# hellosunking/Microcket

Measured on AMD Instinct MI355X. Metric: read-pairs/sec through sam2pairs+dedup (150 bp PE, hg38 names, SAM text resident in HBM), higher is better.
Workload: dtype u8; 1 GPU; C2: 100 M 150 bp PE Micro-C read pairs, hg38, one MI355X -- 100000000 synthetic 150 bp PE read pairs per GPU, hg38 chromosome names, 1 lane(s), unc mode, sam=no, seed 20260105, one step = one pass over the whole resident data set + duplicate marking of the reported pairs on (chr1,pos1,chr2,pos2,strands) + per-chromosome-pair counts; preset=C2, pairs_per_gpu=100000001, sam_bytes_per_gpu=94584442002, block_groups=2097152, blocks=48, parallelism=shard1: independent read-group shards, no data-path collective

## Files before the change

### microcket_amd/csrc/mkt_capi.cpp

```cpp
#include <hip/hip_runtime.h>
#include <stdarg.h>
#include <stdio.h>
#include <stdlib.h>
#include <string.h>
#include <algorithm>
#include <string>
#include <utility>
#include <chrono>
#include <condition_variable>
#include <deque>
#include <mutex>
#include <thread>
#include <vector>

#include "../../include/mkt.h"
#include "mkt_launch.h"

using namespace mkt;

static const size_t kMaxBlock = ((size_t)1 << 31) - 65536;

static thread_local std::string g_create_error;

struct mkt_ctx {
// ... 236 lines not shown

static int ensure_sc_list(mkt_ctx* c, size_t need);

static void set_dims_from_avg(mkt_ctx* c, double bytes_per_line) {
    c->dims_probed = true;
    c->halo_widened = 0;
    if (c->cfg == CFG_SMALL || c->p.tiles != MKT_TILES_AUTO) return;
    c->dims = lean_dims(bytes_per_line);
    if (getenv("MKT_DEBUG_SYNC")) fprintf(stderr, "tile geometry: %.1f bytes per line -> tile %u, halos %u / %u\n", bytes_per_line, c->dims.tile, c->dims.hb, c->dims.hf);
}
static bool shrink_dims(mkt_ctx* c) {
    if (c->cfg == CFG_SMALL || c->dims.tile <= 2048u) return false;
    auto f = [](uint32_t x, uint32_t lo) { uint32_t y = ((uint32_t)(x * 0.6) + 15u) & ~15u; return y < lo ? lo : y; };
    c->dims.tile = f(c->dims.tile, 2048u); c->dims.hb = f(c->dims.hb, 256u); c->dims.hf = f(c->dims.hf, 512u);
    return true;
}
static bool widen_halos(mkt_ctx* c) {
    if (c->cfg == CFG_SMALL || c->halo_widened >= 2) return false;
    const TileDims mx = max_dims();
    auto f = [](uint32_t x, uint32_t hi) { uint32_t y = ((uint32_t)(x * 1.5) + 15u) & ~15u; return y > hi ? hi : y; };
    const uint32_t hb = f(c->dims.hb, mx.hb), hf = f(c->dims.hf, mx.hf);
    const uint32_t delta = (hb - c->dims.hb) + (hf - c->dims.hf);
    if (delta == 0 || c->dims.tile < delta + 2048u) return false;
    c->dims.tile -= delta; c->dims.hb = hb; c->dims.hf = hf;
    ++c->halo_widened;
    if (getenv("MKT_DEBUG_SYNC")) fprintf(stderr, "tile geometry: halos widened -> tile %u, halos %u / %u\n", c->dims.tile, c->dims.hb, c->dims.hf);
    return true;
}
static bool adapt_geometry(mkt_ctx* c, const BlockResult& r) {
    if (c->p.tiles != MKT_TILES_AUTO || c->p.ordered) return false;
    if (r.tiles >= 1000 && (uint64_t)r.pad2 * 500 > r.tiles && widen_halos(c)) return true;
    if (r.tiles >= 8 && (uint64_t)(r.pad - r.pad2) * 8 > r.tiles) return shrink_dims(c);
    return false;
}
static double probe_device_lines(mkt_ctx* c, const uint8_t* d_text, size_t n) {
    const size_t look = n < ((size_t)1 << 20) ? n : ((size_t)1 << 20);
    if (!look) return 0;
    if (!c->d_probe) {
        if (hipMalloc((void**)&c->d_probe, sizeof(unsigned long long)) != hipSuccess) return 0;
        if (hipHostMalloc((void**)&c->h_probe, sizeof(unsigned long long), hipHostMallocDefault) != hipSuccess) return 0;
    }
    if (hipMemsetAsync(c->d_probe, 0, sizeof(unsigned long long), c->stream) != hipSuccess) return 0;
    if (launch_count_newlines(d_text, look, c->d_probe, c->stream) != hipSuccess) return 0;
    if (hipMemcpyAsync(c->h_probe, c->d_probe, sizeof(unsigned long long), hipMemcpyDeviceToHost, c->stream) != hipSuccess) return 0;
    if (hipStreamSynchronize(c->stream) != hipSuccess) return 0;
    return *c->h_probe ? (double)look / (double)*c->h_probe : (double)look;
}
static void smaller_geometry(mkt_ctx* c, const uint8_t* d_text, size_t n) {
    if (c->cfg != CFG_SMALL && d_text) {
        const double avg = probe_device_lines(c, d_text, n);
        const TileDims d = avg > 0 ? lean_dims(avg) : c->dims;
        if (d.tile < c->dims.tile) { c->dims = d; return; }
    }
    if (!shrink_dims(c)) { c->cfg = CFG_SMALL; c->dims = small_dims(); }
}

struct StreamOut { uint8_t* gp; size_t gp_cap; uint8_t* gs; size_t gs_cap; hipEvent_t k0, k1, done; };
static int enqueue_block(mkt_ctx* c, const uint8_t* d_text, size_t n, int cfg, const TileDims& dims, size_t slot, const StreamOut* so = nullptr) {
    if (((uintptr_t)d_text & 15u) != 0) return fail(c, MKT_E_ARG, "block text must be 16-byte aligned");
    if (n >= kMaxBlock) return fail(c, MKT_E_ARG, "block of %zu bytes: must be < 2 GiB - 64 KiB", n);
    const uint32_t ntiles = num_tiles((uint32_t)n, dims.tile);
    int rc = ensure_ws(c, ntiles);
    if (rc) return rc;
    if ((rc = ensure_dev(c, &c->d_pairs, &c->pairs_cap, n / 3 + 65536))) return rc;
    if (c->P.write_sam && (rc = ensure_dev(c, &c->d_sam, &c->sam_cap, n + n / 4 + 65536))) return rc;
    if (!c->d_sc && (rc = ensure_sc_list(c, 1))) return rc;
    KArgs a;
    memset(&a, 0, sizeof a);
    uint8_t* w = c->d_ws;
    a.text = d_text; a.n = (uint32_t)n; a.ntiles = ntiles; a.dims = dims; a.P = c->P;
    a.descA = (uint64_t*)w; w += (size_t)ntiles * 8;
    a.descB = (uint64_t*)w; w += (size_t)ntiles * 8;
    a.descC = (uint64_t*)w; w += (size_t)ntiles * 8;
    a.tile_last = (TileLast*)w; w += (size_t)ntiles * sizeof(TileLast);
    a.tile_groups = (uint64_t*)w; w += (size_t)ntiles * sizeof(uint64_t);
    a.defer_list = (uint32_t*)w;
    w = c->d_ws + ws_tiles_bytes(ntiles);
    a.cur = (RegionCur*)w; w += kMaxRegions * sizeof(RegionCur);
    a.ticket = (uint32_t*)w;
    a.defer_count = (uint32_t*)(w + 64);
    uint32_t* ticket2 = (uint32_t*)(w + 128);
    a.last_tile = (int*)(w + 192);
    a.scan_ticket = (uint32_t*)(w + 224);
    w += 256;
    a.scan_desc = (uint64_t*)w; w += 1024 * sizeof(uint64_t);
    if ((ntiles + finish_chunk_tiles() - 1) / finish_chunk_tiles() > 1024) return fail(c, MKT_E_ARG, "block has too many tiles for the finish scan");
    a.res = (BlockResult*)w;
    a.ordered = c->p.ordered ? 1 : 0;
    a.run = c->d_run;
    a.nregions = c->p.ordered ? 1 : kMaxRegions;
    {
        const size_t need = (size_t)a.nregions * ((n / 256 / (size_t)a.nregions) * 2 + 1024);
        if (c->sc_tmp_cap < need) {
            if (c->d_sc_tmp) { if ((rc = sync_all(c))) return rc; HIPCHK(c, hipFree(c->d_sc_tmp)); }
            c->d_sc_tmp = nullptr; c->sc_tmp_cap = 0;
            HIPCHK(c, hipMalloc((void**)&c->d_sc_tmp, need * sizeof(uint64_t)));
            c->sc_tmp_cap = need;
        }
    }
    a.pairs_rcap = (c->pairs_cap / a.nregions) & ~(uint64_t)15;
    a.sam_rcap = c->P.write_sam ? ((c->sam_cap / a.nregions) & ~(uint64_t)15) : 0;
    a.sc_rcap = c->sc_tmp_cap / a.nregions;
    a.out.pairs = c->d_pairs; a.out.pairs_cap = c->pairs_cap;
    a.out.sam = c->d_sam; a.out.sam_cap = c->P.write_sam ? c->sam_cap : 0;
    a.out.sc = c->d_sc_tmp; a.out.sc_cap = c->sc_tmp_cap;
    a.sc_list = c->d_sc; a.sc_list_cap = c->sc_cap;
    if (c->p.extensions & MKT_EXT_KEYS) {
        if (!c->d_chr) { HIPCHK(c, hipMalloc((void**)&c->d_chr, sizeof(ChrTab))); HIPCHK(c, hipMemsetAsync(c->d_chr, 0, sizeof(ChrTab), c->stream)); }
        const size_t per = (n / 64 / (size_t)a.nregions) * 2 + 4096, need = per * a.nregions;
        if (c->keys_raw_cap < need) {
            if (c->d_keys_raw) { if ((rc = sync_all(c))) return rc; HIPCHK(c, hipFree(c->d_keys_raw)); }
            c->d_keys_raw = nullptr; c->keys_raw_cap = 0;
            HIPCHK(c, hipMalloc((void**)&c->d_keys_raw, need * sizeof(KeyRec)));
            c->keys_raw_cap = need;
        }
        const double per_byte = c->key_density > 0 ? (c->key_density * 2 < 1.0 / 64 ? c->key_density * 2 : 1.0 / 64) : 1.0 / 64;
        const size_t want = (size_t)c->acc.emitted + (size_t)((double)(c->bytes_unsynced + n) * per_byte) + 65536;
        if (c->key_list_cap < want) {
            size_t ncap = c->key_list_cap ? c->key_list_cap * 2 : ((size_t)1 << 22);
            while (ncap < want) ncap *= 2;
            KeyRec* nl = nullptr;
            HIPCHK(c, hipStreamSynchronize(c->stream));
            HIPCHK(c, hipMalloc((void**)&nl, ncap * sizeof(KeyRec)));
            if (c->d_key_list) { HIPCHK(c, hipMemcpy(nl, c->d_key_list, c->key_list_cap * sizeof(KeyRec), hipMemcpyDeviceToDevice)); HIPCHK(c, hipFree(c->d_key_list)); }
            c->d_key_list = nl; c->key_list_cap = ncap;
        }
        a.keys_rcap = c->keys_raw_cap / a.nregions;
        a.out.keys = c->d_keys_raw; a.out.keys_cap = c->keys_raw_cap; a.out.chr = c->d_chr;
        a.out.key_lanes = (c->p.extensions & MKT_EXT_LANES) ? 1u : 0u;
        a.key_list = c->d_key_list; a.key_list_cap = c->key_list_cap;
    }
#if defined(MKT_STAMPS)
    if (!c->d_stamps) { HIPCHK(c, hipMalloc((void**)&c->d_stamps, 16 * sizeof(unsigned long long))); HIPCHK(c, hipMemset(c->d_stamps, 0, 16 * sizeof(unsigned long long))); }
    a.stamps = getenv("MKT_NO_STAMPS") ? nullptr : c->d_stamps;
    { const char* e = getenv("MKT_DEBUG_STOP"); a.debug_stop = e ? atoi(e) : 0; }
#endif
    HIPCHK(c, hipMemsetAsync(c->d_ws, 0, ws_bytes_for(ntiles), c->stream));
    hipEvent_t e0, e1;
    if (so) { e0 = so->k0; e1 = so->k1; }
    else {
        HIPCHK(c, hipEventCreate(&e0));
        HIPCHK(c, hipEventCreate(&e1));
        c->ev.push_back(e0); c->ev.push_back(e1); c->ev_bytes.push_back(n);
    }
    const uint32_t max_wgs = fast_max_workgroups(cfg);
    int grid = (int)(ntiles < max_wgs ? ntiles : max_wgs);
    const bool lean = !c->p.ordered && cfg != CFG_SMALL && !c->no_lean;
    HIPCHK(c, hipEventRecord(e0, c->stream));
    if (lean) {
        HIPCHK(c, launch_fast(a, cfg, grid, c->stream));
        HIPCHK(c, hipEventRecord(e1, c->stream));
        KArgs b = a;
        b.use_list = 1; b.ticket = ticket2;
        HIPCHK(c, launch_tiles(b, cfg, ntiles < 96u ? (int)ntiles : 96, c->stream));
    } else {
        HIPCHK(c, launch_tiles(a, cfg, grid, c->stream));
        HIPCHK(c, hipEventRecord(e1, c->stream));
    }
    HIPCHK(c, launch_finish(a, c->stream));
    if (so) {
        const uint64_t prc = a.nregions > 1 ? a.pairs_rcap : 0, src_ = a.nregions > 1 ? a.sam_rcap : 0;
        HIPCHK(c, launch_gather(a.res, c->d_pairs, prc, so->gp, so->gp_cap, 0, n / 8, c->stream));
        if (c->P.write_sam) HIPCHK(c, launch_gather(a.res, c->d_sam, src_, so->gs, so->gs_cap, 1, n, c->stream));
    }
    HIPCHK(c, hipMemcpyAsync(&c->h_res[slot], a.res, sizeof(BlockResult), hipMemcpyDeviceToHost, c->stream));
    if (so) HIPCHK(c, hipEventRecord(so->done, c->stream));
// ... 1091 lines not shown
```

### microcket_amd/csrc/mkt_kernels.hip

```cpp
#include <hip/hip_runtime.h>
#include <type_traits>
#include "mkt_launch.h"

namespace mkt {

constexpr int NT = 256;
constexpr uint64_t FLAG_AGG = 1ull << 62, FLAG_PREFIX = 2ull << 62, PAYLOAD = (1ull << 62) - 1;
constexpr uint32_t LOOKBACK_SPIN_LIMIT = 1u << 22;

struct ScanScratch { uint64_t a[NT / 64], b[NT / 64]; };

#if defined(MKT_STAMPS)
#define STAMP_DECL() unsigned long long stamp_prev_ = 0, stamp_acc_[16] = {0, 0, 0, 0, 0, 0, 0, 0, 0, 0, 0, 0, 0, 0, 0, 0}
#define STAMP(k)                                                                        \
    do {                                                                                \
        if (tid == 0 && a.stamps) {                                                     \
            const unsigned long long now_ = __builtin_amdgcn_s_memtime();               \
            if ((k) > 0) stamp_acc_[(k)] += now_ - stamp_prev_;                         \
            stamp_prev_ = now_;                                                         \
        }                                                                               \
    } while (0)
#define STAMP_FLUSH(t0_)                                                                \
    do {                                                                                \
        if ((t0_) == 0 && a.stamps) for (int k_ = 1; k_ < 16; ++k_) if (stamp_acc_[k_]) atomicAdd(&a.stamps[k_], stamp_acc_[k_]); \
// ... 101 lines not shown
    const uint32_t y = x & 0x7F7F7F7Fu;
    return ~((y + 0x5F5F5F5Fu) | x) & 0x80808080u;
}
__device__ inline uint32_t pack16(uint32_t f0, uint32_t f1, uint32_t f2, uint32_t f3) {
    const uint32_t lo = __builtin_amdgcn_udot4(f1, 0x80402010u, __builtin_amdgcn_udot4(f0, 0x08040201u, 0u, false), false);
    const uint32_t hi = __builtin_amdgcn_udot4(f3, 0x80402010u, __builtin_amdgcn_udot4(f2, 0x08040201u, 0u, false), false);
    return (lo >> 7) | ((hi >> 7) << 8);
}

__device__ inline uint64_t lookback(uint64_t* desc, uint32_t t, uint64_t agg, uint32_t* err_word) {
    const int lane = threadIdx.x & 63;
    if (t == 0) {
        if (lane == 0) __hip_atomic_store(&desc[0], FLAG_PREFIX | agg, __ATOMIC_RELAXED, __HIP_MEMORY_SCOPE_AGENT);
        return 0;
    }
    if (lane == 0) __hip_atomic_store(&desc[t], FLAG_AGG | agg, __ATOMIC_RELAXED, __HIP_MEMORY_SCOPE_AGENT);
    uint64_t excl = 0;
    int64_t j = (int64_t)t - 1;
    uint32_t spins = 0;
    for (;;) {
        const int64_t idx = j - lane;
        uint64_t w = FLAG_PREFIX;
        if (idx >= 0) w = __hip_atomic_load(&desc[idx], __ATOMIC_RELAXED, __HIP_MEMORY_SCOPE_AGENT);
        const uint32_t flag = (uint32_t)(w >> 62);
        const uint64_t m_prefix = __ballot(flag == 2);
        const uint64_t m_invalid = __ballot(flag == 0);
        const int first = m_prefix ? __builtin_ctzll(m_prefix) : 64;
        const uint64_t needed = first >= 63 ? ~0ull : ((1ull << (first + 1)) - 1);
        if (m_invalid & needed) {
            if (++spins > LOOKBACK_SPIN_LIMIT) { if (lane == 0) atomicOr(err_word, (uint32_t)E_LOOKBACK); break; }
            __builtin_amdgcn_s_sleep(4);
            continue;
        }
        uint64_t c = lane <= first ? (w & PAYLOAD) : 0;
#pragma unroll
        for (int d = 32; d >= 1; d >>= 1) c += shfl_xor64(c, d);
        excl += c;
        if (first < 64) break;
        j -= 64;
    }
    if (lane == 0) __hip_atomic_store(&desc[t], FLAG_PREFIX | ((excl + agg) & PAYLOAD), __ATOMIC_RELAXED, __HIP_MEMORY_SCOPE_AGENT);
    return excl;
}

__device__ inline uint32_t claim_ranges(const KArgs& a, uint32_t region, const TileSums& sums, TileSums& base,
                                        uint32_t& region_pair0, uint32_t& region_sam0, OutPtrs& lim) {
    RegionCur* cur = a.cur + region;
    uint32_t err = 0;
    const uint64_t p0 = (uint64_t)region * a.pairs_rcap, s0 = (uint64_t)region * a.sam_rcap, c0 = (uint64_t)region * a.sc_rcap;
    unsigned long long oa = 0, ob = 0;
    if (sums.pair_bytes | sums.emitted) oa = atomicAdd(&cur->a, (unsigned long long)sums.pair_bytes | ((unsigned long long)sums.emitted << kCurShift));
    if (sums.sam_bytes | sums.sc) ob = atomicAdd(&cur->b, (unsigned long long)sums.sam_bytes | ((unsigned long long)sums.sc << kCurShift));
    const uint64_t op = oa & kCurLow, os = ob & kCurLow, oc = ob >> kCurShift;
    if (op + sums.pair_bytes > a.pairs_rcap) err |= E_PAIRS_CAP;
    if (os + sums.sam_bytes > a.sam_rcap) err |= E_SAM_CAP;
    if (oc + sums.sc > a.sc_rcap) err |= E_SC_CAP;
    base.pair_bytes = (uint32_t)(p0 + op); base.sam_bytes = s0 + os; base.sc = (uint32_t)(c0 + oc);
    base.emitted = (uint32_t)((uint64_t)region * a.keys_rcap + (oa >> kCurShift));
    lim.keys_cap = a.keys_rcap ? ((uint64_t)region * a.keys_rcap + ((oa >> kCurShift) + sums.emitted <= a.keys_rcap ? a.keys_rcap : 0)) : 0;
    region_pair0 = (uint32_t)p0; region_sam0 = (uint32_t)s0;
    lim.pairs_cap = err & E_PAIRS_CAP ? 0 : p0 + a.pairs_rcap;
    lim.sam_cap = err & E_SAM_CAP ? 0 : s0 + a.sam_rcap;
    lim.sc_cap = err & E_SC_CAP ? 0 : c0 + a.sc_rcap;
    return err;
}

template <class Cfg>
__global__ __launch_bounds__(NT) void k_tiles(KArgs a) {
    __shared__ TileState<Cfg> st;
    __shared__ ScanScratch scan;
    __shared__ uint32_t s_tile;
    constexpr int NVEC = (Cfg::W + 15) / 16;
    constexpr int NM16 = Cfg::MW * 4;
    constexpr int VPT = (NVEC + NT - 1) / NT;
    constexpr int IPT = (Cfg::LCAP + NT - 1) / NT;
    const int tid = threadIdx.x;
    const Params P = a.P;
    const uint32_t n = a.n;
    __shared__ OutPtrs s_out;
    const uint32_t region = a.nregions > 1 ? (blockIdx.x & (uint32_t)(a.nregions - 1)) : 0u;
    uint16_t* nlmask = reinterpret_cast<uint16_t*>(st.u.m.nlm);
    uint16_t* wsmask = reinterpret_cast<uint16_t*>(st.u.m.wsm);
    STAMP_DECL();

    for (;;) {
        if (tid == 0) {
            s_out = a.out;
            uint32_t k = atomicAdd(a.ticket, 1u);
            if (a.use_list) k = k < *a.defer_count ? a.defer_list[k] : 0xFFFFFFFFu;
            s_tile = k;
            tile_reset(st);
        }
        __syncthreads();
        const uint32_t t = s_tile;
        if (t >= a.ntiles) break;
        STAMP(0);
        const TileGeom G = tile_geom(t, n, a.dims);
        const uint32_t wlen = G.w1 - G.w0;
        const uint32_t nvec = (wlen + 15u) >> 4;
        const TextView tv = tile_view(st, a.text, n, G);

        constexpr int SPT = (NM16 + NT - 1) / NT;
        uint4 xs[SPT];
#pragma unroll
        for (int q = 0; q < SPT; ++q) {
            const uint32_t v = (uint32_t)tid + (uint32_t)q * NT;
            const uint32_t go = G.w0 + (v << 4);
            xs[q] = *reinterpret_cast<const uint4*>(a.text + ((v < nvec && go + 16u <= n) ? go : 0u));
        }
#pragma unroll
        for (int q = 0; q < SPT; ++q) {
            const uint32_t v = (uint32_t)tid + (uint32_t)q * NT;
            if (v >= (uint32_t)NM16) continue;
            uint32_t mnl = 0, mws = 0;
            if (v < nvec) {
                const uint32_t go = G.w0 + (v << 4);
                uint4 x;
                if (go + 16u <= n) {
                    x = xs[q];
                } else {
                    uint32_t w[4] = {0, 0, 0, 0};
                    for (uint32_t b = 0; go + b < n; ++b) w[b >> 2] |= (uint32_t)a.text[go + b] << ((b & 3u) * 8u);
                    x = make_uint4(w[0], w[1], w[2], w[3]);
                }
                *reinterpret_cast<uint4*>(&st.win[v << 4]) = x;
                mnl = nl_bits(x.x) | (nl_bits(x.y) << 4) | (nl_bits(x.z) << 8) | (nl_bits(x.w) << 12);
                mws = ws_bits(x.x) | (ws_bits(x.y) << 4) | (ws_bits(x.z) << 8) | (ws_bits(x.w) << 12);
                const uint32_t r0 = v << 4;
                if (r0 + 16u > wlen) {
                    const uint32_t keep = wlen - r0;
                    mnl &= (1u << keep) - 1u; mws &= (1u << keep) - 1u;
                }
            } else if (v == nvec && (v << 4) < (uint32_t)(Cfg::W + 16)) {
                *reinterpret_cast<uint4*>(&st.win[v << 4]) = make_uint4(0, 0, 0, 0);
            }
            nlmask[v] = (uint16_t)mnl;
            wsmask[v] = (uint16_t)mws;
        }
        __syncthreads();
        STAMP(1);

        {
            uint64_t cnt = 0, dummy = 0, total, td;
            const uint32_t v0 = tid * VPT;
            auto line_bits = [&](uint32_t v) -> uint32_t {
                uint32_t m = nlmask[v];
                const uint32_t r0 = v << 4;
                if (r0 + 16u > wlen - 1u) { const uint32_t keep = wlen - 1u > r0 ? wlen - 1u - r0 : 0u; m &= keep >= 16u ? 0xFFFFu : ((1u << keep) - 1u); }
                return m;
            };
            for (uint32_t k = 0; k < (uint32_t)VPT; ++k) if (v0 + k < nvec) cnt += __popc(line_bits(v0 + k));
            uint64_t ex = cnt;
            block_exscan2(ex, dummy, total, td, scan);
            const uint32_t lead = G.w0 == 0 ? 1u : 0u;
            const uint32_t NL = (uint32_t)total + lead;
            if (NL > (uint32_t)Cfg::LCAP) {
                if (tid == 0) { lds_or(&st.err, E_LINE_TABLE); st.NL = 0; st.first_idx = 0; st.end_idx = 0; }
            } else {
                uint32_t idx = (uint32_t)ex + lead;
                for (uint32_t k = 0; k < (uint32_t)VPT; ++k) {
                    if (v0 + k >= nvec) break;
                    uint32_t m = line_bits(v0 + k);
                    while (m) {
                        const uint32_t b = __builtin_ctz(m);
                        st.off[idx++] = G.w0 + ((v0 + k) << 4) + b + 1u;
                        m &= m - 1u;
// ... 423 lines not shown
        }
        if (total && st.base.pair_bytes + total <= s_out.pairs_cap) {
            const auto& g = st.u.g;
            for (uint32_t e = (ltid + (uint32_t)(NTW / 2)) & (uint32_t)(NTW - 1); e < st.sums.emitted; e += NTW) {
                const uint32_t i = g.em_idx[e];
                fast_emit_line(st, g.g_slot[i], g.g_plen[i], dst + g.x_pair[i]);
            }
        }
        __syncthreads();
        STAMP(11);
        if (tid < (int)C_COUNT) wg_cnt[tid] += st.cnt[tid];
        if (tid == 0 && (st.abn >> 8)) atomicOr(&a.res->err, st.abn >> 8);
        const bool sam_copy = P.write_sam && st.sums.sam_bytes && st.base.sam_bytes + st.sums.sam_bytes <= s_out.sam_cap;
        uint32_t* eo = st.rc.f.pos;
        uint32_t* es = st.rc.f.rclip;
        uint32_t E = 0;
        if (sam_copy) {
            E = (uint32_t)(__popcll(st.m_emit[0]) + __popcll(st.m_emit[1]) + __popcll(st.m_emit[2]) + __popcll(st.m_emit[3]));
            for (uint32_t i = first_idx + (uint32_t)tid; i < NLe; i += NTW) {
                if (!mask_bit(st.m_emit, i)) continue;
                uint32_t k = (uint32_t)__popcll(st.m_emit[i >> 6] & ((1ull << (i & 63u)) - 1ull));
                for (uint32_t w = 0; w < (i >> 6); ++w) k += (uint32_t)__popcll(st.m_emit[w]);
                eo[k] = st.u.g.x_sam[i];
                es[k] = st.goff[i];
            }
            if (tid == 0) eo[E] = (uint32_t)st.sums.sam_bytes;
        }
        if (P.write_sam) __syncthreads();
        if (sam_copy && E) {
            const uint32_t total = (uint32_t)st.sums.sam_bytes;
            uint8_t* dbase = s_out.sam + st.base.sam_bytes;
            const uint8_t* tbase = a.text + G.w0;
            auto line_of = [&](uint32_t d) {
                uint32_t lo = 0, hi = E - 1u;
                while (lo < hi) { const uint32_t mid = (lo + hi + 1u) >> 1; if (eo[mid] <= d) lo = mid; else hi = mid - 1u; }
                return lo;
            };
            const uint32_t head0 = (uint32_t)((16u - ((uintptr_t)dbase & 15u)) & 15u);
            const uint32_t head = head0 < total ? head0 : total;
            const uint32_t nv = (total - head) >> 4, tail0 = head + (nv << 4);
            if ((uint32_t)tid < head) { const uint32_t k = line_of((uint32_t)tid); *MKT_GLOBAL(uint8_t, dbase + tid) = tbase[es[k] + (uint32_t)tid - eo[k]]; }
            if ((uint32_t)tid < total - tail0) { const uint32_t d = tail0 + (uint32_t)tid, k = line_of(d); *MKT_GLOBAL(uint8_t, dbase + d) = tbase[es[k] + d - eo[k]]; }
            for (uint32_t v = (uint32_t)tid; v < nv; v += NTW) {
                const uint32_t d = head + (v << 4);
                const uint32_t k = line_of(d);
                const uint32_t o = d - eo[k], left = eo[k + 1u] - d;
                const uint32_t so = es[k] + o;
                uint4 x;
                if (left >= 16u) __builtin_memcpy(&x, tbase + so, 16);
                else if (k + 2u <= E && eo[k + 2u] - eo[k + 1u] >= 16u - left && (uint64_t)G.w0 + so + 16u <= (uint64_t)n) {
                    uint4 xa, xb;
                    __builtin_memcpy(&xa, tbase + so, 16);
                    __builtin_memcpy(&xb, tbase + es[k + 1u] - left, 16);
                    const uint32_t* pa = reinterpret_cast<const uint32_t*>(&xa);
                    const uint32_t* pb = reinterpret_cast<const uint32_t*>(&xb);
                    uint32_t* px = reinterpret_cast<uint32_t*>(&x);
#pragma unroll
                    for (uint32_t q = 0; q < 4u; ++q) {
                        const uint32_t m = left >= 4u * q + 4u ? 0xFFFFFFFFu : (left <= 4u * q ? 0u : (1u << (8u * (left - 4u * q))) - 1u);
                        px[q] = (pa[q] & m) | (pb[q] & ~m);
                    }
                } else {
                    uint32_t q0 = 0, q1 = 0, q2 = 0, q3 = 0;
                    uint32_t kk = k, oo = so, lim = left;
#pragma unroll
                    for (uint32_t b2 = 0; b2 < 16u; ++b2) {
                        while (lim == 0u) { ++kk; oo = es[kk]; lim = eo[kk + 1u] - eo[kk]; }
                        const uint32_t by = (uint32_t)tbase[oo++] << (8u * (b2 & 3u));
                        if (b2 < 4u) q0 |= by; else if (b2 < 8u) q1 |= by; else if (b2 < 12u) q2 |= by; else q3 |= by;
                        --lim;
                    }
                    x = make_uint4(q0, q1, q2, q3);
                }
                *MKT_GLOBAL(uint4, dbase + d) = x;
            }
        }
        __syncthreads();
        STAMP(8);
    }
    if (tid0 < (int)C_COUNT && wg_cnt[tid0]) atomicAdd(&a.res->counters[tid0], wg_cnt[tid0]);
    STAMP_FLUSH(tid0);
}

constexpr int NTF = 1024;
__global__ __launch_bounds__(NTF) void k_finish_scan(KArgs a) {
    __shared__ uint64_t s_wave[NTF / 64];
    __shared__ uint64_t s_pre;
    __shared__ uint32_t s_chunk;
    const int tid = threadIdx.x, lane = tid & 63, wv = tid >> 6;
    if (tid == 0) s_chunk = atomicAdd(a.scan_ticket, 1u);
    __syncthreads();
    const uint32_t chunk = s_chunk;
    const uint32_t t = chunk * NTF + tid;
    const uint64_t x = t < a.ntiles ? a.tile_groups[t] : 0ull;
    if (t < a.ntiles && a.tile_last[t].valid) atomicMax(a.last_tile, (int)t + 1);
    uint64_t inc = x;
#pragma unroll
    for (int d = 1; d < 64; d <<= 1) { uint64_t y = shfl_up64(inc, d); if (lane >= d) inc += y; }
    if (lane == 63) s_wave[wv] = inc;
    __syncthreads();
    uint64_t pre = 0, tot = 0;
    for (int w = 0; w < NTF / 64; ++w) { if (w < wv) pre += s_wave[w]; tot += s_wave[w]; }
    if (wv == 0) {
        const uint64_t ex = lookback(a.scan_desc, chunk, ((tot & 0x7FFFFFFFull) << 31) | (tot >> 32), &a.res->err);
        if (lane == 0) s_pre = (ex >> 31) | ((ex & 0x7FFFFFFFull) << 32);
    }
    __syncthreads();
    if (t < a.ntiles) a.tile_groups[t] = s_pre + pre + inc - x;
    if (chunk == gridDim.x - 1 && tid == 0) a.res->groups = (s_pre + tot) & 0xFFFFFFFFull;
}

constexpr int kFinishGrid = 16;
__global__ __launch_bounds__(NTF) void k_finish(KArgs a) {
    const int tid = threadIdx.x;
    BlockResult* r = a.res;
    __shared__ uint64_t s_scpre[kMaxRegions + 1], s_ca[kMaxRegions], s_cb[kMaxRegions];
    __shared__ uint32_t s_err;
    if (tid < a.nregions) { s_ca[tid] = a.cur[tid].a; s_cb[tid] = a.cur[tid].b; }
    __syncthreads();
    if (tid == 0) {
        uint64_t pb = 0, em = 0, sb = 0, sc = 0;
        uint32_t err = 0;
        for (int q = 0; q < a.nregions; ++q) {
            const uint64_t ca = s_ca[q], cb = s_cb[q];
            const uint64_t p = ca & kCurLow, e = ca >> kCurShift, sm = cb & kCurLow, c = cb >> kCurShift;
            if (blockIdx.x == 0) { r->rpair[q] = p; r->rsam[q] = sm; }
            s_scpre[q] = sc;
            pb += p; em += e; sb += sm; sc += c;
            if (!a.ordered) {
                if (p > a.pairs_rcap) err |= E_PAIRS_CAP;
                if (sm > a.sam_rcap) err |= E_SAM_CAP;
                if (c > a.sc_rcap) err |= E_SC_CAP;
            }
        }
        s_scpre[a.nregions] = sc;
        if (a.ordered) { if (pb > a.out.pairs_cap) err |= E_PAIRS_CAP; if (sb > a.out.sam_cap) err |= E_SAM_CAP; if (sc > a.out.sc_cap) err |= E_SC_CAP; }
        if (a.run->sc + sc > a.sc_list_cap) err |= E_SC_CAP;
        if (a.keys_rcap && a.run->emitted + em > a.key_list_cap) err |= E_SC_CAP;
        s_err = err | r->err;
        if (blockIdx.x == 0) {
            r->pair_bytes = pb; r->emitted = em; r->sam_bytes = sb; r->sc = sc; r->nregions = (uint32_t)a.nregions;
            r->pad = a.defer_count ? *a.defer_count : 0u;
            r->pad2 = a.defer_count ? a.defer_count[1] : 0u;
            r->tiles = a.ntiles;
            const int last = *a.last_tile - 1;
            if (last >= 0) r->last = a.tile_last[last];
        }
    }
    __syncthreads();
    if (s_err == 0) {
        const uint64_t sc_base = a.run->sc, g_base = a.run->groups;
        const int nr = a.nregions;
        const int parts = (int)gridDim.x >= nr ? (int)gridDim.x / nr : 1;
        for (int q = (int)blockIdx.x % nr; q < nr; q += (int)gridDim.x) {
            const int part = (int)blockIdx.x / nr;
            if (part >= parts) break;
            const uint64_t cnt = s_scpre[q + 1] - s_scpre[q];
            const uint64_t* src = a.out.sc + (uint64_t)q * (a.ordered ? 0 : a.sc_rcap);
            for (uint64_t k = (uint64_t)part * NTF + tid; k < cnt; k += (uint64_t)parts * NTF) {
                const uint64_t e = src[k];
                a.sc_list[sc_base + s_scpre[q] + k] = g_base + (a.tile_groups[(uint32_t)(e >> 32)] & 0xFFFFFFFFull) + (uint32_t)(e & 0xFFFFFFFFu);
            }
        }
    }
    __syncthreads();
    if (blockIdx.x == 0 && tid == 0 && (s_err & ~r->err)) r->err |= s_err;
}

__global__ __launch_bounds__(256) void k_keys_place(KArgs a) {
    const BlockResult* r = a.res;
    if (r->err) return;
    __shared__ uint64_t pre[kMaxRegions + 1];
    if (threadIdx.x == 0) {
        uint64_t acc = 0;
        for (int q = 0; q < kMaxRegions; ++q) { pre[q] = acc; if (q < a.nregions) acc += a.cur[q].a >> kCurShift; }
        pre[kMaxRegions] = acc;
    }
    __syncthreads();
    const uint64_t base = a.run->emitted, total = pre[kMaxRegions];
    const uint64_t rstride = a.ordered ? 0 : a.keys_rcap;
    for (uint64_t x = (uint64_t)blockIdx.x * blockDim.x + threadIdx.x; x < total; x += (uint64_t)gridDim.x * blockDim.x) {
        uint32_t q = 0;
#pragma unroll
        for (uint32_t k = 1; k < (uint32_t)kMaxRegions; ++k) q += (x >= pre[k]) ? 1u : 0u;
        KeyRec rec = a.out.keys[(uint64_t)q * rstride + (x - pre[q])];
        const uint64_t ord = base + (a.tile_groups[(uint32_t)(rec.ord >> 16)] >> 32) + (rec.ord & 0xFFFFu);
        rec.ord = ord;
        a.key_list[ord] = rec;
    }
}
__global__ void k_run_advance(KArgs a) {
    BlockResult* r = a.res;
    if (threadIdx.x == 0 && r->err == 0) { a.run->groups += r->groups; a.run->sc += r->sc; a.run->emitted += r->emitted; }
}

struct GatherArgs {
    const BlockResult* res;
    const uint8_t* src; uint64_t rcap;
    uint8_t* dst; uint64_t dst_cap;
    int32_t which;
};
__global__ __launch_bounds__(256) void k_gather(GatherArgs g) {
    __shared__ uint64_t pre[kMaxRegions + 1];
    __shared__ uint64_t s_hole, s_tp;
    const BlockResult* r = g.res;
    if (r->err) return;
    if (threadIdx.x == 0) {
        const uint32_t nr = r->nregions ? r->nregions : 1u;
        uint64_t acc = 0;
        for (uint32_t q = 0; q < (uint32_t)kMaxRegions; ++q) { pre[q] = acc; if (q < nr) acc += g.which ? r->rsam[q] : r->rpair[q]; }
        pre[kMaxRegions] = acc;
        uint64_t tp = 0, hole = acc;
        if (r->last.valid) {
            tp = g.which ? r->last.sam_bytes : r->last.pair_bytes;
            const uint32_t lr = r->last.region < nr ? r->last.region : 0u;
            hole = pre[lr] + (g.which ? r->last.sam_off : r->last.pair_off);
        }
        s_hole = hole; s_tp = tp;
    }
    __syncthreads();
    const uint64_t total = pre[kMaxRegions], tp = s_tp, hole = s_hole, body = total - tp;
    if (total > g.dst_cap) return;
    auto src_of = [&](uint64_t x) -> const uint8_t* {
        const uint64_t y = x < body ? (x < hole ? x : x + tp) : hole + (x - body);
        uint32_t q = 0;
#pragma unroll
        for (uint32_t k = 1; k < (uint32_t)kMaxRegions; ++k) q += (y >= pre[k]) ? 1u : 0u;
        return g.src + (uint64_t)q * g.rcap + (y - pre[q]);
    };
    for (uint64_t x0 = ((uint64_t)blockIdx.x * blockDim.x + threadIdx.x) * 16u; x0 < total; x0 += (uint64_t)gridDim.x * blockDim.x * 16u) {
        const uint64_t x1 = x0 + 15u < total ? x0 + 15u : total - 1u;
        const uint8_t* a = src_of(x0);
        const uint8_t* b = src_of(x1);
        if (x1 - x0 == 15u && (uint64_t)(b - a) == 15u) {
            uint4 v;
            __builtin_memcpy(&v, a, 16);
            *reinterpret_cast<uint4*>(g.dst + x0) = v;
        } else {
            for (uint64_t x = x0; x <= x1; ++x) g.dst[x] = *src_of(x);
        }
    }
}
hipError_t launch_gather(const BlockResult* d_res, const uint8_t* src, uint64_t rcap, uint8_t* dst, uint64_t dst_cap, int which, uint64_t max_bytes, hipStream_t s) {
    GatherArgs g;
    g.res = d_res; g.src = src; g.rcap = rcap; g.dst = dst; g.dst_cap = dst_cap; g.which = which;
    uint64_t chunks = (max_bytes + 15) / 16;
    unsigned grid = (unsigned)((chunks + 255) / 256 < 2048 ? (chunks + 255) / 256 : 2048);
    if (grid == 0) grid = 1;
    hipLaunchKernelGGL(k_gather, dim3(grid), dim3(256), 0, s, g);
    return hipGetLastError();
}

__global__ void k_sc_logged(const uint64_t* list, uint64_t n, uint64_t drop_group, uint64_t group_offset, uint64_t K_total, uint32_t ref_threads,
                            unsigned long long* out) {
    unsigned long long mine = 0;
    for (uint64_t k = (uint64_t)blockIdx.x * blockDim.x + threadIdx.x; k < n; k += (uint64_t)gridDim.x * blockDim.x) {
        const uint64_t g = list[k];
        if (g == drop_group) continue;
        if (selfcircle_logged(group_offset + g, K_total, ref_threads)) ++mine;
    }
    for (int d = 32; d >= 1; d >>= 1) mine += shfl_xor64(mine, d);
    if ((threadIdx.x & 63) == 0 && mine) atomicAdd(out, mine);
}
hipError_t launch_sc_logged(const uint64_t* list, uint64_t n, uint64_t drop_group, uint64_t group_offset, uint64_t K_total, uint32_t ref_threads,
                            unsigned long long* out, hipStream_t s) {
    if (n == 0) return hipSuccess;
    const unsigned grid = (unsigned)((n + 255) / 256 < 1024 ? (n + 255) / 256 : 1024);
    hipLaunchKernelGGL(k_sc_logged, dim3(grid), dim3(256), 0, s, list, n, drop_group, group_offset, K_total, ref_threads, out);
    return hipGetLastError();
}

typedef FastCfg<kLeanTile, kLeanHB, kLeanHF, kLeanLCAP> CfgLean;
typedef TileCfg<kLeanTile, kLeanHB, kLeanHF, 512, 4> CfgFast;
typedef TileCfg<256, 64, 192, 512, 4> CfgSmall;

TileDims small_dims() { return cfg_dims<CfgSmall>(); }
TileDims max_dims() { return cfg_dims<CfgLean>(); }
static bool dims_ok(const TileDims& d, const TileDims& mx) {
    return d.tile >= 16u && !((d.tile | d.hb | d.hf) & 15u) && d.tile <= mx.tile && d.hb <= mx.hb && d.hf <= mx.hf;
}

uint32_t fast_max_workgroups(int) { return 256u * 4u; }

hipError_t launch_tiles(const KArgs& a, int cfg, int grid, hipStream_t s) {
    if (a.ntiles == 0) return hipSuccess;
    if (!dims_ok(a.dims, cfg == CFG_SMALL ? small_dims() : max_dims())) return hipErrorInvalidValue;
    if (cfg == CFG_SMALL) hipLaunchKernelGGL(k_tiles<CfgSmall>, dim3(grid), dim3(NT), 0, s, a);
    else hipLaunchKernelGGL(k_tiles<CfgFast>, dim3(grid), dim3(NT), 0, s, a);
    return hipGetLastError();
}
hipError_t launch_fast(const KArgs& a, int, int grid, hipStream_t s) {
    if (a.ntiles == 0) return hipSuccess;
    if (!dims_ok(a.dims, max_dims())) return hipErrorInvalidValue;
    hipLaunchKernelGGL((k_fast<CfgLean, NT, 2, 4>), dim3(grid), dim3(NT), 0, s, a);
    return hipGetLastError();
}
__global__ void k_count_nl(const uint8_t* text, size_t n, unsigned long long* out) {
    unsigned long long mine = 0;
    const size_t nv = n >> 4;
    for (size_t v = (size_t)blockIdx.x * blockDim.x + threadIdx.x; v < nv; v += (size_t)gridDim.x * blockDim.x) {
        const uint4 x = reinterpret_cast<const uint4*>(text)[v];
        mine += __popc(nl_flags(x.x)) + __popc(nl_flags(x.y)) + __popc(nl_flags(x.z)) + __popc(nl_flags(x.w));
    }
    if (blockIdx.x == 0 && threadIdx.x == 0) for (size_t b = nv << 4; b < n; ++b) mine += text[b] == '\n';
    for (int d = 32; d >= 1; d >>= 1) mine += shfl_xor64(mine, d);
    if ((threadIdx.x & 63) == 0 && mine) atomicAdd(out, mine);
}
hipError_t launch_count_newlines(const uint8_t* text, size_t n, unsigned long long* out, hipStream_t s) {
    if (n) hipLaunchKernelGGL(k_count_nl, dim3(64), dim3(256), 0, s, text, n, out);
    return hipGetLastError();
}
hipError_t launch_finish(const KArgs& a, hipStream_t s) {
    const unsigned chunks = (a.ntiles + NTF - 1) / NTF;
    if (chunks) hipLaunchKernelGGL(k_finish_scan, dim3(chunks), dim3(NTF), 0, s, a);
    hipLaunchKernelGGL(k_finish, dim3(kFinishGrid), dim3(NTF), 0, s, a);
    if (a.keys_rcap) hipLaunchKernelGGL(k_keys_place, dim3(2048), dim3(256), 0, s, a);
    hipLaunchKernelGGL(k_run_advance, dim3(1), dim3(64), 0, s, a);
    return hipGetLastError();
}
uint32_t finish_chunk_tiles() { return NTF; }

constexpr int DD_WG = 256;
constexpr int DS_WG = 512;
constexpr int DS_NW = DS_WG / 64;
constexpr int DS_T = 8192;
constexpr int DS_K = DS_T / DS_WG;
constexpr int DS_D = 7, DS_R = 1 << DS_D;
constexpr int DS_SCAN_WG = 1024, DS_SCAN_V = 8;
constexpr uint64_t kKeyMask1 = 0xFFFFFFFFC000FFFFull;
static_assert(DS_R == 2 * 64, "the scatter's prologue gives each lane of wave 0 two digits");

__device__ inline bool key_eq(const KeyRec& x, const KeyRec& y) { return x.k0 == y.k0 && (x.k1 & kKeyMask1) == (y.k1 & kKeyMask1); }

__global__ __launch_bounds__(DS_WG) void k_dd_prep(const KeyRec* keys, uint64_t n, int ib, uint64_t* rec, uint32_t* cnt, uint32_t G) {
    __shared__ uint32_t c[DS_R];
    if (threadIdx.x < DS_R) c[threadIdx.x] = 0;
    __syncthreads();
    const uint64_t b = (uint64_t)blockIdx.x * DS_T, e = b + DS_T < n ? b + DS_T : n, hi = ~((1ull << ib) - 1ull);
    for (uint64_t j = b + threadIdx.x; j < e; j += DS_WG) {
        const uint64_t r = (mix64(keys[j].k0 ^ mix64(keys[j].k1 & kKeyMask1)) & hi) | j;
        rec[j] = r;
        atomicAdd(&c[(r >> ib) & (DS_R - 1)], 1u);
    }
    __syncthreads();
    if (threadIdx.x < DS_R) cnt[threadIdx.x * G + blockIdx.x] = c[threadIdx.x];
}
__global__ __launch_bounds__(DS_WG) void k_dd_count(const uint64_t* rec, uint64_t n, int shift, uint32_t* cnt, uint32_t G) {
    __shared__ uint32_t c[DS_R];
    if (threadIdx.x < DS_R) c[threadIdx.x] = 0;
    __syncthreads();
    const uint64_t b = (uint64_t)blockIdx.x * DS_T, m = (b + DS_T < n ? b + DS_T : n) - b;
    const ulonglong2* v = reinterpret_cast<const ulonglong2*>(rec + b);
    for (uint64_t i = threadIdx.x; i < m / 2; i += DS_WG) {
        const ulonglong2 x = v[i];
        atomicAdd(&c[(x.x >> shift) & (DS_R - 1)], 1u);
        atomicAdd(&c[(x.y >> shift) & (DS_R - 1)], 1u);
    }
    if ((m & 1) && threadIdx.x == 0) atomicAdd(&c[(rec[b + m - 1] >> shift) & (DS_R - 1)], 1u);
    __syncthreads();
    if (threadIdx.x < DS_R) cnt[threadIdx.x * G + blockIdx.x] = c[threadIdx.x];
}
__global__ __launch_bounds__(DS_SCAN_WG) void k_dd_dscan(uint32_t* cnt, uint32_t G, uint32_t* tot) {
    __shared__ uint32_t wsum[DS_SCAN_WG / 64];
    const int lane = threadIdx.x & 63, wv = threadIdx.x >> 6;
    uint32_t* row = cnt + (uint64_t)blockIdx.x * G;
    uint32_t carry = 0;
    for (uint32_t base = 0; base < G; base += DS_SCAN_WG * DS_SCAN_V) {
        const uint32_t i0 = base + threadIdx.x * DS_SCAN_V;
        uint32_t v[DS_SCAN_V], s = 0;
#pragma unroll
        for (int k = 0; k < DS_SCAN_V; ++k) { v[k] = i0 + k < G ? row[i0 + k] : 0u; s += v[k]; }
        const uint32_t inc = wave_iscan32(s);
        if (lane == 63) wsum[wv] = inc;
        __syncthreads();
        uint32_t pre = carry, all = 0;
#pragma unroll
        for (int w = 0; w < DS_SCAN_WG / 64; ++w) { const uint32_t x = wsum[w]; if (w < wv) pre += x; all += x; }
        pre += inc - s;
#pragma unroll
        for (int k = 0; k < DS_SCAN_V; ++k) { if (i0 + k < G) row[i0 + k] = pre; pre += v[k]; }
        carry += all;
        __syncthreads();
    }
    if (threadIdx.x == 0) tot[blockIdx.x] = carry;
}
__global__ __launch_bounds__(DS_WG, 4) void k_dd_scatter(const uint64_t* rec, uint64_t n, int shift, const uint32_t* cnt, const uint32_t* tot, uint32_t G, uint64_t* rec2) {
    __shared__ uint64_t tile[DS_T];
    __shared__ uint32_t wrun[DS_NW][DS_R];
    __shared__ uint32_t gdelta[DS_R];
    const int tid = threadIdx.x, lane = tid & 63, wv = tid >> 6;
    const uint64_t b = (uint64_t)blockIdx.x * DS_T, m = (b + DS_T < n ? b + DS_T : n) - b;
    uint32_t gc0 = 0, gc1 = 0, t0 = 0, t1 = 0;
    if (wv == 0) {
        gc0 = cnt[(uint64_t)(2 * lane) * G + blockIdx.x]; gc1 = cnt[(uint64_t)(2 * lane + 1) * G + blockIdx.x];
        t0 = tot[2 * lane]; t1 = tot[2 * lane + 1];
    }
    for (int i = tid; i < DS_NW * DS_R; i += DS_WG) (&wrun[0][0])[i] = 0u;
    __syncthreads();
    uint64_t r[DS_K];
    uint32_t loc[DS_K / 2];
    const uint64_t lt = (1ull << lane) - 1ull;
#pragma unroll
    for (int k = 0; k < DS_K; ++k) {
// ... 318 lines not shown
```

### microcket_amd/csrc/mkt_launch.h

```cpp
#pragma once
#include <hip/hip_runtime.h>
#include "mkt_host.h"
#include "mkt_fast.h"
#include "mkt_synth.h"

namespace mkt {

enum { CFG_FAST = 0, CFG_SMALL = 1 };

struct DevRun { uint64_t groups, sc, emitted; };

struct alignas(128) RegionCur { unsigned long long a, b; unsigned long long pad[14]; };
constexpr int kMaxRegions = 16;
constexpr int kCurShift = 36;
constexpr unsigned long long kCurLow = (1ull << kCurShift) - 1ull;

struct KArgs {
    const uint8_t* text;
    uint32_t n;
    uint32_t ntiles;
    TileDims dims;
    Params P;
    uint64_t* descA;
    uint64_t* descB;
    uint64_t* descC;
    uint32_t* ticket;
    uint64_t* tile_groups;
    int32_t ordered;
    TileLast* tile_last;
    uint32_t* defer_list;
    uint32_t* defer_count;
    int* last_tile;
    uint64_t* scan_desc;
    uint32_t* scan_ticket;
    int32_t use_list;
    BlockResult* res;
    DevRun* run;
    RegionCur* cur;
    int32_t nregions;
    uint64_t pairs_rcap, sam_rcap, sc_rcap;
    uint64_t* sc_list;
    uint64_t sc_list_cap;
    uint64_t keys_rcap;
    KeyRec* key_list;
    uint64_t key_list_cap;
    OutPtrs out;
    unsigned long long* stamps;
    int32_t debug_stop;
};

TileDims small_dims();
TileDims max_dims();
uint32_t fast_max_workgroups(int cfg);
hipError_t launch_count_newlines(const uint8_t* text, size_t n, unsigned long long* out, hipStream_t s);
hipError_t launch_tiles(const KArgs& a, int cfg, int grid, hipStream_t s);
hipError_t launch_fast(const KArgs& a, int cfg, int grid, hipStream_t s);
uint32_t finish_chunk_tiles();
hipError_t launch_finish(const KArgs& a, hipStream_t s);
hipError_t launch_gather(const BlockResult* d_res, const uint8_t* src, uint64_t rcap, uint8_t* dst, uint64_t dst_cap, int which, uint64_t max_bytes, hipStream_t s);
hipError_t launch_sc_logged(const uint64_t* list, uint64_t n, uint64_t drop_group, uint64_t group_offset, uint64_t K_total, uint32_t ref_threads,
                            unsigned long long* out, hipStream_t s);

struct DedupResult { uint64_t total, dups; };
hipError_t launch_dedup(const KeyRec* keys, uint64_t n, uint8_t* flags, void* work, size_t work_bytes, DedupResult* d_res, hipStream_t s);
size_t dedup_work_bytes(uint64_t n);
size_t partition_work_bytes();
hipError_t launch_partition(const KeyRec* keys, uint64_t n, const uint16_t* d_lut, uint32_t world, uint32_t* hist, KeyRec* send, uint32_t* perm, uint32_t* G_out, hipStream_t s);
hipError_t launch_unpermute(const uint8_t* in, const uint32_t* perm, uint64_t n, uint8_t* out, unsigned long long* dups, hipStream_t s);
hipError_t launch_chrstat(const KeyRec* keys, uint64_t n, const uint16_t* dense_of_slot, uint32_t ndense, unsigned long long* counts, hipStream_t s);

hipError_t launch_synth_sizes(const SynParams& p, uint64_t first, uint64_t n, uint64_t* sizes, hipStream_t s);
hipError_t launch_exscan(uint64_t* v, uint64_t n, uint64_t* total, hipStream_t s);
hipError_t launch_synth_write(const SynParams& p, uint64_t first, uint64_t n, const uint64_t* offs, char* out, hipStream_t s);
hipError_t launch_synth_tail(const SynParams& p, char* out, hipStream_t s);
size_t synth_tail_bytes(const SynParams& p);

}
```

Baseline: 2.061 billion read-pairs/s.

## Fuse per-block finish kernels into scan-with-epilogue and single place kernel

```diff
diff --git a/microcket_amd/csrc/mkt_capi.cpp b/microcket_amd/csrc/mkt_capi.cpp
--- a/microcket_amd/csrc/mkt_capi.cpp
+++ b/microcket_amd/csrc/mkt_capi.cpp
@@ -342,6 +342,8 @@
     uint32_t* ticket2 = (uint32_t*)(w + 128);
     a.last_tile = (int*)(w + 192);
     a.scan_ticket = (uint32_t*)(w + 224);
+    a.run_base = (uint64_t*)(w + 8);
+    a.end_count = (uint32_t*)(w + 240);
     w += 256;
     a.scan_desc = (uint64_t*)w; w += 1024 * sizeof(uint64_t);
     if ((ntiles + finish_chunk_tiles() - 1) / finish_chunk_tiles() > 1024) return fail(c, MKT_E_ARG, "block has too many tiles for the finish scan");
diff --git a/microcket_amd/csrc/mkt_kernels.hip b/microcket_amd/csrc/mkt_kernels.hip
--- a/microcket_amd/csrc/mkt_kernels.hip
+++ b/microcket_amd/csrc/mkt_kernels.hip
@@ -207,6 +207,7 @@
     uint16_t* nlmask = reinterpret_cast<uint16_t*>(st.u.m.nlm);
     uint16_t* wsmask = reinterpret_cast<uint16_t*>(st.u.m.wsm);
     STAMP_DECL();
+    if (a.use_list && blockIdx.x >= *a.defer_count) return;
 
     for (;;) {
         if (tid == 0) {
@@ -796,116 +797,139 @@
     STAMP_FLUSH(tid0);
 }
 
-constexpr int NTF = 1024;
-__global__ __launch_bounds__(NTF) void k_finish_scan(KArgs a) {
-    __shared__ uint64_t s_wave[NTF / 64];
+constexpr int NTE = 256;
+constexpr uint32_t kEndChunk = 1024;
+constexpr uint32_t kPlaceGrid = 2048;
+
+__device__ inline void drain_vmem() { asm volatile("s_waitcnt vmcnt(0)" ::: "memory"); }
+
+__device__ inline uint32_t region_of(uint64_t x, const uint64_t* pre) {
+    uint32_t q = 0;
+#pragma unroll
+    for (uint32_t k = 1; k < (uint32_t)kMaxRegions; ++k) q += (x >= pre[k]) ? 1u : 0u;
+    return q;
+}
+
+__global__ __launch_bounds__(NTE) void k_block_scan(KArgs a) {
+    __shared__ uint64_t s_wave[NTE / 64];
+    __shared__ uint64_t s_ca[kMaxRegions], s_cb[kMaxRegions];
     __shared__ uint64_t s_pre;
-    __shared__ uint32_t s_chunk;
+    __shared__ uint32_t s_ticket, s_last;
     const int tid = threadIdx.x, lane = tid & 63, wv = tid >> 6;
-    if (tid == 0) s_chunk = atomicAdd(a.scan_ticket, 1u);
-    __syncthreads();
-    const uint32_t chunk = s_chunk;
-    const uint32_t t = chunk * NTF + tid;
-    const uint64_t x = t < a.ntiles ? a.tile_groups[t] : 0ull;
-    if (t < a.ntiles && a.tile_last[t].valid) atomicMax(a.last_tile, (int)t + 1);
-    uint64_t inc = x;
-#pragma unroll
-    for (int d = 1; d < 64; d <<= 1) { uint64_t y = shfl_up64(inc, d); if (lane >= d) inc += y; }
-    if (lane == 63) s_wave[wv] = inc;
-    __syncthreads();
-    uint64_t pre = 0, tot = 0;
-    for (int w = 0; w < NTF / 64; ++w) { if (w < wv) pre += s_wave[w]; tot += s_wave[w]; }
-    if (wv == 0) {
-        const uint64_t ex = lookback(a.scan_desc, chunk, ((tot & 0x7FFFFFFFull) << 31) | (tot >> 32), &a.res->err);
-        if (lane == 0) s_pre = (ex >> 31) | ((ex & 0x7FFFFFFFull) << 32);
-    }
-    __syncthreads();
-    if (t < a.ntiles) a.tile_groups[t] = s_pre + pre + inc - x;
-    if (chunk == gridDim.x - 1 && tid == 0) a.res->groups = (s_pre + tot) & 0xFFFFFFFFull;
-}
-
-constexpr int kFinishGrid = 16;
-__global__ __launch_bounds__(NTF) void k_finish(KArgs a) {
-    const int tid = threadIdx.x;
     BlockResult* r = a.res;
-    __shared__ uint64_t s_scpre[kMaxRegions + 1], s_ca[kMaxRegions], s_cb[kMaxRegions];
-    __shared__ uint32_t s_err;
-    if (tid < a.nregions) { s_ca[tid] = a.cur[tid].a; s_cb[tid] = a.cur[tid].b; }
-    __syncthreads();
+    const int nr = a.nregions;
+    const uint32_t chunks = (a.ntiles + kEndChunk - 1u) / kEndChunk;
+    if (tid == 0) s_ticket = atomicAdd(a.scan_ticket, 1u);
+    if (tid < nr) { s_ca[tid] = a.cur[tid].a; s_cb[tid] = a.cur[tid].b; }
+    __syncthreads();
+    const uint32_t chunk = s_ticket;
+    if (chunk < chunks) {
+        const uint32_t t0 = chunk * kEndChunk + (uint32_t)tid * 4u;
+        uint64_t x[4];
+        int lastv = 0;
+#pragma unroll
+        for (uint32_t k = 0; k < 4u; ++k) {
+            const uint32_t t = t0 + k;
+            x[k] = t < a.ntiles ? a.tile_groups[t] : 0ull;
+            if (t < a.ntiles && a.tile_last[t].valid) lastv = (int)t + 1;
+        }
+#pragma unroll
+        for (int d = 32; d >= 1; d >>= 1) { const int o = __shfl_xor(lastv, d, 64); lastv = o > lastv ? o : lastv; }
+        if (lane == 0 && lastv) atomicMax(a.last_tile, lastv);
+        const uint64_t own = x[0] + x[1] + x[2] + x[3];
+        uint64_t inc = own;
+#pragma unroll
+        for (int d = 1; d < 64; d <<= 1) { const uint64_t y = shfl_up64(inc, d); if (lane >= d) inc += y; }
+        if (lane == 63) s_wave[wv] = inc;
+        __syncthreads();
+        uint64_t pre = 0, tot = 0;
+#pragma unroll
+        for (int w = 0; w < NTE / 64; ++w) { if (w < wv) pre += s_wave[w]; tot += s_wave[w]; }
+        if (wv == 0) {
+            const uint64_t ex = lookback(a.scan_desc, chunk, ((tot & 0x7FFFFFFFull) << 31) | (tot >> 32), &r->err);
+            if (lane == 0) s_pre = (ex >> 31) | ((ex & 0x7FFFFFFFull) << 32);
+        }
+        __syncthreads();
+        uint64_t v = s_pre + pre + inc - own;
+#pragma unroll
+        for (uint32_t k = 0; k < 4u; ++k) {
+            const uint32_t t = t0 + k;
+            if (t < a.ntiles) a.tile_groups[t] = v;
+            v += x[k];
+        }
+        if (chunk == chunks - 1u && tid == 0)
+            __hip_atomic_store(MKT_GLOBAL(uint64_t, &r->groups), (s_pre + tot) & 0xFFFFFFFFull, __ATOMIC_RELAXED, __HIP_MEMORY_SCOPE_AGENT);
+    }
     if (tid == 0) {
-        uint64_t pb = 0, em = 0, sb = 0, sc = 0;
-        uint32_t err = 0;
-        for (int q = 0; q < a.nregions; ++q) {
-            const uint64_t ca = s_ca[q], cb = s_cb[q];
-            const uint64_t p = ca & kCurLow, e = ca >> kCurShift, sm = cb & kCurLow, c = cb >> kCurShift;
-            if (blockIdx.x == 0) { r->rpair[q] = p; r->rsam[q] = sm; }
-            s_scpre[q] = sc;
-            pb += p; em += e; sb += sm; sc += c;
-            if (!a.ordered) {
-                if (p > a.pairs_rcap) err |= E_PAIRS_CAP;
-                if (sm > a.sam_rcap) err |= E_SAM_CAP;
-                if (c > a.sc_rcap) err |= E_SC_CAP;
-            }
-        }
-        s_scpre[a.nregions] = sc;
-        if (a.ordered) { if (pb > a.out.pairs_cap) err |= E_PAIRS_CAP; if (sb > a.out.sam_cap) err |= E_SAM_CAP; if (sc > a.out.sc_cap) err |= E_SC_CAP; }
-        if (a.run->sc + sc > a.sc_list_cap) err |= E_SC_CAP;
-        if (a.keys_rcap && a.run->emitted + em > a.key_list_cap) err |= E_SC_CAP;
-        s_err = err | r->err;
-        if (blockIdx.x == 0) {
-            r->pair_bytes = pb; r->emitted = em; r->sam_bytes = sb; r->sc = sc; r->nregions = (uint32_t)a.nregions;
-            r->pad = a.defer_count ? *a.defer_count : 0u;
-            r->pad2 = a.defer_count ? a.defer_count[1] : 0u;
-            r->tiles = a.ntiles;
-            const int last = *a.last_tile - 1;
-            if (last >= 0) r->last = a.tile_last[last];
-        }
-    }
-    __syncthreads();
-    if (s_err == 0) {
-        const uint64_t sc_base = a.run->sc, g_base = a.run->groups;
-        const int nr = a.nregions;
-        const int parts = (int)gridDim.x >= nr ? (int)gridDim.x / nr : 1;
-        for (int q = (int)blockIdx.x % nr; q < nr; q += (int)gridDim.x) {
-            const int part = (int)blockIdx.x / nr;
-            if (part >= parts) break;
-            const uint64_t cnt = s_scpre[q + 1] - s_scpre[q];
-            const uint64_t* src = a.out.sc + (uint64_t)q * (a.ordered ? 0 : a.sc_rcap);
-            for (uint64_t k = (uint64_t)part * NTF + tid; k < cnt; k += (uint64_t)parts * NTF) {
-                const uint64_t e = src[k];
-                a.sc_list[sc_base + s_scpre[q] + k] = g_base + (a.tile_groups[(uint32_t)(e >> 32)] & 0xFFFFFFFFull) + (uint32_t)(e & 0xFFFFFFFFu);
-            }
-        }
-    }
-    __syncthreads();
-    if (blockIdx.x == 0 && tid == 0 && (s_err & ~r->err)) r->err |= s_err;
-}
-
-__global__ __launch_bounds__(256) void k_keys_place(KArgs a) {
+        drain_vmem();
+        s_last = __hip_atomic_fetch_add(MKT_GLOBAL(uint32_t, a.end_count), 1u, __ATOMIC_RELAXED, __HIP_MEMORY_SCOPE_AGENT) == gridDim.x - 1u;
+    }
+    __syncthreads();
+    if (!s_last || tid != 0) return;
+    __builtin_amdgcn_fence(__ATOMIC_ACQUIRE, "agent");
+    drain_vmem();
+    uint64_t pb = 0, em = 0, sb = 0, sc = 0;
+    uint32_t err = 0;
+    for (int q = 0; q < nr; ++q) {
+        const uint64_t ca = s_ca[q], cb = s_cb[q];
+        const uint64_t p = ca & kCurLow, e = ca >> kCurShift, sm = cb & kCurLow, c = cb >> kCurShift;
+        r->rpair[q] = p; r->rsam[q] = sm;
+        pb += p; em += e; sb += sm; sc += c;
+        if (!a.ordered) {
+            if (p > a.pairs_rcap) err |= E_PAIRS_CAP;
+            if (sm > a.sam_rcap) err |= E_SAM_CAP;
+            if (c > a.sc_rcap) err |= E_SC_CAP;
+        }
+        if (a.keys_rcap && e > a.keys_rcap) err |= E_SC_CAP;
+    }
+    if (a.ordered) { if (pb > a.out.pairs_cap) err |= E_PAIRS_CAP; if (sb > a.out.sam_cap) err |= E_SAM_CAP; if (sc > a.out.sc_cap) err |= E_SC_CAP; }
+    const uint64_t g0 = a.run->groups, sc0 = a.run->sc, em0 = a.run->emitted;
+    if (sc0 + sc > a.sc_list_cap) err |= E_SC_CAP;
+    if (a.keys_rcap && em0 + em > a.key_list_cap) err |= E_SC_CAP;
+    r->pair_bytes = pb; r->emitted = em; r->sam_bytes = sb; r->sc = sc; r->nregions = (uint32_t)nr;
+    r->pad = a.defer_count ? *a.defer_count : 0u;
+    r->pad2 = a.defer_count ? a.defer_count[1] : 0u;
+    r->tiles = a.ntiles;
+    const int last = __hip_atomic_load(MKT_GLOBAL(int, a.last_tile), __ATOMIC_RELAXED, __HIP_MEMORY_SCOPE_AGENT) - 1;
+    if (last >= 0) r->last = a.tile_last[last];
+    err |= __hip_atomic_load(MKT_GLOBAL(uint32_t, &r->err), __ATOMIC_RELAXED, __HIP_MEMORY_SCOPE_AGENT);
+    if (err) { atomicOr(&r->err, err); return; }
+    a.run_base[0] = g0; a.run_base[1] = sc0; a.run_base[2] = em0;
+    const uint64_t groups = __hip_atomic_load(MKT_GLOBAL(uint64_t, &r->groups), __ATOMIC_RELAXED, __HIP_MEMORY_SCOPE_AGENT);
+    a.run->groups = g0 + groups; a.run->sc = sc0 + sc; a.run->emitted = em0 + em;
+}
+
+__global__ __launch_bounds__(NTE) void k_block_place(KArgs a) {
     const BlockResult* r = a.res;
     if (r->err) return;
-    __shared__ uint64_t pre[kMaxRegions + 1];
+    __shared__ uint64_t s_kpre[kMaxRegions + 1], s_scpre[kMaxRegions + 1];
     if (threadIdx.x == 0) {
-        uint64_t acc = 0;
-        for (int q = 0; q < kMaxRegions; ++q) { pre[q] = acc; if (q < a.nregions) acc += a.cur[q].a >> kCurShift; }
-        pre[kMaxRegions] = acc;
-    }
-    __syncthreads();
-    const uint64_t base = a.run->emitted, total = pre[kMaxRegions];
-    const uint64_t rstride = a.ordered ? 0 : a.keys_rcap;
-    for (uint64_t x = (uint64_t)blockIdx.x * blockDim.x + threadIdx.x; x < total; x += (uint64_t)gridDim.x * blockDim.x) {
-        uint32_t q = 0;
-#pragma unroll
-        for (uint32_t k = 1; k < (uint32_t)kMaxRegions; ++k) q += (x >= pre[k]) ? 1u : 0u;
-        KeyRec rec = a.out.keys[(uint64_t)q * rstride + (x - pre[q])];
-        const uint64_t ord = base + (a.tile_groups[(uint32_t)(rec.ord >> 16)] >> 32) + (rec.ord & 0xFFFFu);
-        rec.ord = ord;
-        a.key_list[ord] = rec;
-    }
-}
-__global__ void k_run_advance(KArgs a) {
-    BlockResult* r = a.res;
-    if (threadIdx.x == 0 && r->err == 0) { a.run->groups += r->groups; a.run->sc += r->sc; a.run->emitted += r->emitted; }
+        uint64_t em = 0, sc = 0;
+        for (int q = 0; q < kMaxRegions; ++q) {
+            s_kpre[q] = em; s_scpre[q] = sc;
+            if (q < a.nregions) { em += a.cur[q].a >> kCurShift; sc += a.cur[q].b >> kCurShift; }
+        }
+        s_kpre[kMaxRegions] = em; s_scpre[kMaxRegions] = sc;
+    }
+    __syncthreads();
+    const uint64_t g_base = a.run_base[0], sc_base = a.run_base[1], k_base = a.run_base[2];
+    const uint64_t stride = (uint64_t)gridDim.x * blockDim.x, x0 = (uint64_t)blockIdx.x * blockDim.x + threadIdx.x;
+    if (a.keys_rcap) {
+        const uint64_t total = s_kpre[kMaxRegions], rstride = a.ordered ? 0 : a.keys_rcap;
+        for (uint64_t x = x0; x < total; x += stride) {
+            const uint32_t q = region_of(x, s_kpre);
+            KeyRec rec = a.out.keys[(uint64_t)q * rstride + (x - s_kpre[q])];
+            const uint64_t ord = k_base + (a.tile_groups[(uint32_t)(rec.ord >> 16)] >> 32) + (rec.ord & 0xFFFFu);
+            rec.ord = ord;
+            a.key_list[ord] = rec;
+        }
+    }
+    const uint64_t total = s_scpre[kMaxRegions], sstride = a.ordered ? 0 : a.sc_rcap;
+    for (uint64_t x = x0; x < total; x += stride) {
+        const uint32_t q = region_of(x, s_scpre);
+        const uint64_t e = a.out.sc[(uint64_t)q * sstride + (x - s_scpre[q])];
+        a.sc_list[sc_base + x] = g_base + (a.tile_groups[(uint32_t)(e >> 32)] & 0xFFFFFFFFull) + (uint32_t)(e & 0xFFFFFFFFu);
+    }
 }
 
 struct GatherArgs {
@@ -1025,14 +1049,12 @@
     return hipGetLastError();
 }
 hipError_t launch_finish(const KArgs& a, hipStream_t s) {
-    const unsigned chunks = (a.ntiles + NTF - 1) / NTF;
-    if (chunks) hipLaunchKernelGGL(k_finish_scan, dim3(chunks), dim3(NTF), 0, s, a);
-    hipLaunchKernelGGL(k_finish, dim3(kFinishGrid), dim3(NTF), 0, s, a);
-    if (a.keys_rcap) hipLaunchKernelGGL(k_keys_place, dim3(2048), dim3(256), 0, s, a);
-    hipLaunchKernelGGL(k_run_advance, dim3(1), dim3(64), 0, s, a);
+    const uint32_t chunks = (a.ntiles + kEndChunk - 1u) / kEndChunk;
+    hipLaunchKernelGGL(k_block_scan, dim3(chunks ? chunks : 1u), dim3(NTE), 0, s, a);
+    hipLaunchKernelGGL(k_block_place, dim3(kPlaceGrid), dim3(NTE), 0, s, a);
     return hipGetLastError();
 }
-uint32_t finish_chunk_tiles() { return NTF; }
+uint32_t finish_chunk_tiles() { return kEndChunk; }
 
 constexpr int DD_WG = 256;
 constexpr int DS_WG = 512;
diff --git a/microcket_amd/csrc/mkt_launch.h b/microcket_amd/csrc/mkt_launch.h
--- a/microcket_amd/csrc/mkt_launch.h
+++ b/microcket_amd/csrc/mkt_launch.h
@@ -33,6 +33,8 @@
     int* last_tile;
     uint64_t* scan_desc;
     uint32_t* scan_ticket;
+    uint32_t* end_count;
+    uint64_t* run_base;
     int32_t use_list;
     BlockResult* res;
     DevRun* run;
```

Result: faster. 2.087 billion read-pairs/s, median of 6 (+1.2%).
